# DaanVrancken/HubbardTN

Hardware: AMD Instinct MI355X
Metric: DMRG sweep time (s) + GS energy/site, 1-band Hubbard L=64 chi=1024 (lower is better)
Workload: dtype c128; 1 GPU; one-band Hubbard chain L=64 U/t=4, half filling, fZ2xSU(2)xU(1), two-site DMRG sweep (2L-3=125 bond updates) at chi=1024 (TensorKit dim units); model=one_band, L=64, chi=1024, krylovdim=30, parallelism=sector-parallel apply x1, backend=hip

## Files before the change

hubbardtn_amd/csrc/htn_svd.hip:

```cpp
#include <algorithm>
#include <utility>
#include <vector>

#include "htn_common.h"

#define JAC_THREADS 1024
#define JAC_MAXEL 8

template <int GS>
__device__ __forceinline__ double group_sum(double v) {
    v = row_sum16(v);
    if (GS == 16) return v;
    const double a = lane_bcast<0>(v) + lane_bcast<16>(v);
    const double b = lane_bcast<32>(v) + lane_bcast<48>(v);
    if (GS == 32) return (threadIdx.x & 32) ? b : a;
    return a + b;
}

template <int GS>
__device__ __forceinline__ double jacobi_pair(double2* ga, double2* gb, double2* __restrict__ va,
                                              double2* __restrict__ vb, int m, int n, int sub, double tol,
                                              bool accumulate, double zero2) {
    double2 a[JAC_MAXEL], b[JAC_MAXEL];
    double aa = 0.0, bb = 0.0, gr = 0.0, gi = 0.0;
// ... 1651 lines not shown
__device__ __forceinline__ void ring_send(const double2* __restrict__ src, double2* slot, int cnt, int tid, bool local) {
    const __amdgpu_buffer_rsrc_t rs = __builtin_amdgcn_make_buffer_rsrc((void*)slot, 0, cnt * 16, 0x00020000);
    if (local) {
        for (int idx = tid; idx < cnt; idx += RING_THREADS) {
            const double2 v = src[idx];
            ring_u4 u;
            __builtin_memcpy(&u, &v, 16);
            __builtin_amdgcn_raw_buffer_store_b128(u, rs, idx * 16, 0, 0);
        }
    } else {
        for (int idx = tid; idx < cnt; idx += RING_THREADS) {
            const double2 v = src[idx];
            ring_u4 u;
            __builtin_memcpy(&u, &v, 16);
            __builtin_amdgcn_raw_buffer_store_b128(u, rs, idx * 16, 0, 16);
        }
    }
}
__device__ __forceinline__ void ring_flag(unsigned* flag, unsigned epoch, bool local) {
    if (local) __hip_atomic_store(flag, epoch, __ATOMIC_RELAXED, __HIP_MEMORY_SCOPE_WORKGROUP);
    else __hip_atomic_store(flag, epoch, __ATOMIC_RELAXED, __HIP_MEMORY_SCOPE_AGENT);
}
__device__ __forceinline__ void ring_recv(double2* dst, const double2* slot, int cnt, int tid) {
    const __amdgpu_buffer_rsrc_t rs = __builtin_amdgcn_make_buffer_rsrc((void*)slot, 0, cnt * 16, 0x00020000);
#define RING_LD(q) const ring_u4 u##q = __builtin_amdgcn_raw_buffer_load_b128(rs, (tid + q * RING_THREADS) * 16, 0, 16)
    RING_LD(0);
    RING_LD(1);
    RING_LD(2);
    RING_LD(3);
    RING_LD(4);
    RING_LD(5);
    RING_LD(6);
    RING_LD(7);
    RING_LD(8);
#undef RING_LD
    auto put = [&](int idx, ring_u4 u) {
        if (idx < cnt) {
            double2 v;
            __builtin_memcpy(&v, &u, 16);
            dst[idx] = v;
        }
    };
    put(tid + 0 * RING_THREADS, u0);
    put(tid + 1 * RING_THREADS, u1);
    put(tid + 2 * RING_THREADS, u2);
    put(tid + 3 * RING_THREADS, u3);
    put(tid + 4 * RING_THREADS, u4);
    put(tid + 5 * RING_THREADS, u5);
    put(tid + 6 * RING_THREADS, u6);
    put(tid + 7 * RING_THREADS, u7);
    put(tid + 8 * RING_THREADS, u8);
}

template <int GS, int E, bool NORMS>
__device__ __forceinline__ double ring_rotate(double2 (&a)[E], const double2 (&b)[E], double2* b_out, double& aa, double& bb,
                                              double tol2, double zero2) {
    double gr = 0.0, gi = 0.0;
    if (NORMS) {
        double sa = 0.0, sb = 0.0;
#pragma unroll
        for (int e = 0; e < E; ++e) {
            sa = fma(a[e].x, a[e].x, fma(a[e].y, a[e].y, sa));
            sb = fma(b[e].x, b[e].x, fma(b[e].y, b[e].y, sb));
        }
        aa = group_sum<GS>(sa);
        bb = group_sum<GS>(sb);
    }
#pragma unroll
    for (int e = 0; e < E; ++e) {
        gr = fma(a[e].x, b[e].x, fma(a[e].y, b[e].y, gr));
        gi = fma(a[e].x, b[e].y, fma(-a[e].y, b[e].x, gi));
    }
    gr = group_sum<GS>(gr);
    gi = group_sum<GS>(gi);
    if (aa <= zero2 || bb <= zero2) return 0.0;
    const double g2 = fma(gr, gr, gi * gi);
    const double ab = aa * bb;
    if (g2 == 0.0) return 0.0;
    const double ratio2 = g2 * __builtin_amdgcn_rcp(ab);
    if (g2 <= tol2 * ab) return ratio2;
    const double h = bb - aa;
    const double w2 = fma(h, h, 4.0 * g2);
    const double w = w2 * __builtin_amdgcn_rsq(w2);
    double q = 2.0 * __builtin_amdgcn_rcp(fabs(h) + w);
    q = h >= 0.0 ? q : -q;
    const double c = fast_rsq(fma(q * q, g2, 1.0));
    const double cq = c * q;
    const double sr = cq * gr, si = -cq * gi;
    aa = fma(-q, g2, aa);
    bb = fma(q, g2, bb);
#pragma unroll
    for (int e = 0; e < E; ++e) {
        double2 nb;
        nb.x = fma(si, a[e].y, fma(sr, a[e].x, c * b[e].x));
        nb.y = fma(-si, a[e].x, fma(sr, a[e].y, c * b[e].y));
        b_out[GS * e] = nb;
        double x = a[e].x * c, y = a[e].y * c;
        x = fma(-sr, b[e].x, x);
        y = fma(-sr, b[e].y, y);
        a[e].x = fma(si, b[e].y, x);
        a[e].y = fma(-si, b[e].x, y);
    }
    return ratio2;
}

struct RingStamps {
    long long t[6];
};
#if defined(HTN_RING_STEP_PROF) && !defined(HTN_RING_PROF)
#error "HTN_RING_STEP_PROF needs HTN_RING_PROF (the split is stored with the phase times)"
#endif
#ifdef HTN_RING_STEP_PROF
#define RING_ST(st, i)                                                                                      \
    do {                                                                                                    \
        __builtin_amdgcn_sched_barrier(0);                                                                  \
        asm volatile("s_memtime %0\n\ts_waitcnt lgkmcnt(0)" : "=s"((st).t[i])::"memory");                  \
        __builtin_amdgcn_sched_barrier(0);                                                                  \
    } while (0)
#else
#define RING_ST(st, i) \
    do {               \
    } while (0)
#endif

template <int GS, int E>
__device__ __forceinline__ double ring_rotate_scaled(double2 (&a)[E], const double2 (&b)[E], double2* b_out, double& aa, double& bb,
                                                     double& sa, double& sb, double tol2, double zero2, RingStamps& st) {
    double gr = 0.0, gi = 0.0, gr1 = 0.0, gi1 = 0.0;
#pragma unroll
    for (int e = 0; e + 1 < E; e += 2) {
        gr = fma(a[e].x, b[e].x, fma(a[e].y, b[e].y, gr));
        gi = fma(a[e].x, b[e].y, fma(-a[e].y, b[e].x, gi));
        gr1 = fma(a[e + 1].x, b[e + 1].x, fma(a[e + 1].y, b[e + 1].y, gr1));
        gi1 = fma(a[e + 1].x, b[e + 1].y, fma(-a[e + 1].y, b[e + 1].x, gi1));
    }
    if (E & 1) {
        gr = fma(a[E - 1].x, b[E - 1].x, fma(a[E - 1].y, b[E - 1].y, gr));
        gi = fma(a[E - 1].x, b[E - 1].y, fma(-a[E - 1].y, b[E - 1].x, gi));
    }
    gr = group_sum<GS>(gr + gr1);
    gi = group_sum<GS>(gi + gi1);
    RING_ST(st, 2);
    if (aa <= zero2 || bb <= zero2) return 0.0;
    const double ss = sa * sb;
    const double g2 = ss * ss * fma(gr, gr, gi * gi);
    const double ab = aa * bb;
    if (g2 == 0.0) return 0.0;
    const double ratio2 = g2 * __builtin_amdgcn_rcp(ab);
    if (g2 <= tol2 * ab) return ratio2;
    const double h = bb - aa;
    const double w2 = fma(h, h, 4.0 * g2);
    const double w = w2 * __builtin_amdgcn_rsq(w2);
    double q = 2.0 * __builtin_amdgcn_rcp(fabs(h) + w);
    q = h >= 0.0 ? q : -q;
    const double c = fast_rsq(fma(q * q, g2, 1.0));
    aa = fma(-q, g2, aa);
    bb = fma(q, g2, bb);
    const double qb = q * sb * sb, qa = q * sa * sa;
    const double mur = qb * gr, mui = -qb * gi;
    const double nur = qa * gr, nui = qa * gi;
    sa *= c;
    sb *= c;
    RING_ST(st, 3);
#pragma unroll
    for (int e = 0; e < E; ++e) {
        double2 nb;
        nb.x = fma(-nui, a[e].y, fma(nur, a[e].x, b[e].x));
        nb.y = fma(nui, a[e].x, fma(nur, a[e].y, b[e].y));
        b_out[GS * e] = nb;
    }
#pragma unroll
    for (int e = 0; e < E; ++e) {
        double x = fma(-mur, b[e].x, a[e].x), y = fma(-mur, b[e].y, a[e].y);
        a[e].x = fma(mui, b[e].y, x);
        a[e].y = fma(-mui, b[e].x, y);
    }
    RING_ST(st, 4);
    return ratio2;
}

template <int GS, int E, bool TWO>
__device__ __forceinline__ double ring_cross(double2* T, double2* B, int nt, int nb, int tid, double tol2, double zero2, double* bnorm,
                                             double* bscale, long long* split) {
    static_assert(!TWO || GS == 16, "two partners per step need both rows of a pair in one wave");
    constexpr int mp = GS * E;
    const int grp = tid / GS, sub = tid % GS;
    const int wm = nt > nb ? nt : nb;
    double ratio = 0.0;
    if (nt == 0 || nb == 0) return ratio;
    const bool own = grp < nt;
    double2 a[E];
    double aa = 0.0, sa = 1.0;
    if (own) {
#pragma unroll
        for (int e = 0; e < E; ++e) a[e] = T[grp * mp + sub + GS * e];
        double t = 0.0;
#pragma unroll
        for (int e = 0; e < E; ++e) t = fma(a[e].x, a[e].x, fma(a[e].y, a[e].y, t));
        aa = group_sum<GS>(t);
    }
    if (grp < nb) {
        const double2* bc = B + grp * mp + sub;
        double sb = 0.0;
#pragma unroll
        for (int e = 0; e < E; ++e) {
            const double2 v = bc[GS * e];
            sb = fma(v.x, v.x, fma(v.y, v.y, sb));
        }
        sb = group_sum<GS>(sb);
        if (sub == 0) {
            bnorm[grp] = sb;
            bscale[grp] = 1.0;
        }
    }
    __syncthreads();
    constexpr int phases = TWO ? 2 : 1;
    const int hp = TWO ? (wm + 1) >> 1 : wm;
    const int row = TWO ? (grp & 1) : 0, pr = TWO ? (grp >> 1) : grp;
    (void)split;
    for (int s = 0; s < hp; ++s) {
        int jp = pr + s;
        jp = jp >= hp ? jp - hp : jp;
#ifdef HTN_RING_STEP_PROF
        long long acc[4] = {0, 0, 0, 0};
        bool all = true;
#endif
        RingStamps st;
#pragma unroll
        for (int ph = 0; ph < phases; ++ph) {
            const int j = TWO ? 2 * jp + (row ^ ph) : jp;
            st.t[4] = 0;
            RING_ST(st, 0);
            if (own && j < nb) {
                double2 b[E];
                double2* bc = B + j * mp + sub;
#pragma unroll
                for (int e = 0; e < E; ++e) b[e] = bc[GS * e];
                double bb = bnorm[j], sb = bscale[j];
                RING_ST(st, 1);
                const double rr = ring_rotate_scaled<GS, E>(a, b, bc, aa, bb, sa, sb, tol2, zero2, st);
                ratio = rr > ratio ? rr : ratio;
                if (sub == 0) {
                    bnorm[j] = bb;
                    bscale[j] = sb;
                }
            }
#ifdef HTN_RING_STEP_PROF
            if (st.t[4] == 0) all = false;
            else {
                acc[0] += st.t[1] - st.t[0];
                acc[1] += st.t[2] - st.t[1];
                acc[2] += st.t[3] - st.t[2];
                acc[3] += st.t[4] - st.t[3];
            }
#endif
            if (TWO && ph == 0) asm volatile("s_waitcnt lgkmcnt(0)" ::: "memory");
        }
#ifdef HTN_RING_STEP_PROF
        const long long tb = st.t[4];
#endif
        __syncthreads();
#ifdef HTN_RING_STEP_PROF
        RING_ST(st, 5);
        if (tid == 0 && all && tb != 0) {
            for (int q = 0; q < 4; ++q) split[q] += acc[q];
            split[4] += st.t[5] - tb;
            split[5] += 1;
            split[6] += phases;
        }
#endif
    }
    if (own) {
#pragma unroll
        for (int e = 0; e < E; ++e) T[grp * mp + sub + GS * e] = make_double2(a[e].x * sa, a[e].y * sa);
    }
    if (grp < nb) {
        const double sb = bscale[grp];
        if (sb != 1.0) {
            double2* bc = B + grp * mp + sub;
#pragma unroll
            for (int e = 0; e < E; ++e) {
                const double2 v = bc[GS * e];
                bc[GS * e] = make_double2(v.x * sb, v.y * sb);
            }
        }
    }
    __syncthreads();
    return ratio;
}

template <int GS, int E>
__device__ __forceinline__ double ring_intra(double2* T, int nt, double2* B, int nb, int tid, double tol2, double zero2) {
    constexpr int mp = GS * E;
    const int grp = tid / GS, sub = tid % GS;
    const int npT = nt + (nt & 1), npB = nb + (nb & 1), hT = npT >> 1, hB = npB >> 1;
    const int steps = (npT > npB ? npT : npB) - 1;
    double ratio = 0.0;
    for (int r = 0; r < steps; ++r) {
        double2* base = nullptr;
        int np = 0, pn = 0, p = 0;
        if (grp < hT) base = T, np = npT, pn = nt, p = grp;
        else if (grp < hT + hB) base = B, np = npB, pn = nb, p = grp - hT;
        if (base && r < np - 1) {
            const int md = np - 1;
            int i, j;
            if (p == 0) i = np - 1, j = r;
            else {
                i = r + p;
                i = i >= md ? i - md : i;
                j = r + md - p;
                j = j >= md ? j - md : j;
            }
            if (i < pn && j < pn) {
                const int lo = i < j ? i : j, hi = i < j ? j : i;
                const double rr = jacobi_pair_pad<GS, E>(base + lo * mp, base + hi * mp, sub, tol2, zero2);
                ratio = rr > ratio ? rr : ratio;
            }
        }
        __syncthreads();
    }
    return ratio;
}

#ifdef HTN_RING_PROF
__device__ long long g_ring_prof[256 * 16];
extern "C" int htn_ring_prof_dump(long long* out) {
    HIP_TRY(hipDeviceSynchronize());
    HIP_TRY(hipMemcpyFromSymbol(out, HIP_SYMBOL(g_ring_prof), sizeof(long long) * 256 * 16));
    return 0;
}
#define RING_T(var) const long long var = wall_clock64()
#define RING_ACC(slot, a, b) prof[slot] += (b) - (a)
#else
#define RING_T(var)
#define RING_ACC(slot, a, b)
#endif
struct RingArgs {
    double2* Vj;
    double2* G;
    double* S;
    const htn_svd_block* desc;
    const int* large_ids;
    const RingItem* items;
    const int* perm;
    const double* zero2;
    double2* mbox;
    unsigned* sync;
    int arrive_off, fail_off, conv_off;
    int xcc_off;
    int max_sweeps;
    int two_partner;
    double tol;
    int* info;
    int* sweeps_out;
};

template <int GS, int E>
__device__ __forceinline__ void ring_run(const RingArgs A, const RingItem it, const htn_svd_block D, double2* lds, int* s_top, int* s_bot,
                         unsigned long long* s_rbits, int* s_ok, double* s_bnorm, int* s_local) {
    constexpr int mp = GS * E;
    const int tid = threadIdx.x, lane = tid & 63, wave = tid >> 6;
    const int P = it.P, k = it.k, w = it.w, n = it.n, m = D.m;
    double2* __restrict__ X = A.Vj + D.v_off;
    const int slot_elems = w * mp;
    double2* bufT = lds;
    double2* bufB = lds + slot_elems;
    unsigned* flags = A.sync;
    unsigned* fail = A.sync + A.fail_off;
    const double zero2 = A.zero2[it.li];
    const double tol2 = A.tol * A.tol, thr = fmax(tol2, 0.1 * A.tol);
    auto ncols = [&](int q) {
        const int c = n - q * w;
        return c < 0 ? 0 : (c > w ? w : c);
    };
    if (tid < P) {
        s_top[tid] = 2 * tid;
        s_bot[tid] = 2 * tid + 1;
    }
    if (tid == 0) {
        *s_ok = 1;
        int local = 0;
        if (P > 1 && A.xcc_off >= 0) {
            unsigned xcc;
            asm volatile("s_getreg_b32 %0, hwreg(HW_REG_XCC_ID)" : "=s"(xcc));
            xcc = (xcc & 0xfu) + 1u;
            unsigned* xw = A.sync + A.xcc_off + it.g0;
            __hip_atomic_store(xw + k, xcc, __ATOMIC_RELAXED, __HIP_MEMORY_SCOPE_AGENT);
            local = 1;
            for (int q = 0; q < P && local >= 0; ++q) {
                if (!ring_wait_ge(xw + q, 1u, fail)) local = -1;
                else if (__hip_atomic_load(xw + q, __ATOMIC_RELAXED, __HIP_MEMORY_SCOPE_AGENT) != xcc) local = local > 0 ? 0 : local;
            }
            if (local < 0) *s_ok = 0;
        }
        *s_local = local > 0 ? 1 : 0;
    }
    __syncthreads();
    const bool local = *s_local != 0;
    {
        const int gsx = m <= 16 * JAC_MAXEL ? 16 : (m <= 32 * JAC_MAXEL ? 32 : 64);
        const int ldx = gsx * ((m + gsx - 1) / gsx);
        for (int side = 0; side < 2; ++side) {
            const int q = side ? s_bot[k] : s_top[k];
            double2* buf = side ? bufB : bufT;
            const int cnt = ncols(q) * mp;
            for (int idx = tid; idx < cnt; idx += RING_THREADS) {
                const int c = idx / mp, i = idx - c * mp;
                buf[idx] = i < m ? X[(int64_t)(q * w + c) * ldx + i] : make_double2(0.0, 0.0);
            }
        }
    }
    __syncthreads();
#ifdef HTN_RING_PROF
    long long prof[16] = {0, 0, 0, 0, 0, 0, 0, 0, 0, 0, 0, 0, 0, 0, 0, 0};
    const long long prof_t0 = wall_clock64();
    long long prof_c0;
    asm volatile("s_memtime %0\n\ts_waitcnt lgkmcnt(0)" : "=s"(prof_c0)::"memory");
#endif
    long long* split = nullptr;
#ifdef HTN_RING_STEP_PROF
    split = prof + 8;
#endif
    int sweeps = 0;
    bool done = n < 2, ok = *s_ok != 0;
    const int rounds = 2 * P - 1;
    while (!done && ok && sweeps < A.max_sweeps) {
        double ratio = 0.0;
        for (int r = 0; r < rounds && ok; ++r) {
            const unsigned epoch = (unsigned)(sweeps * rounds + r + 1);
            const int par = (int)(epoch & 1u);
            const int nt = ncols(s_top[k]), nb = ncols(s_bot[k]);
            RING_T(p0);
            double rr;
            if constexpr (GS == 16) {
                if (A.two_partner) rr = ring_cross<GS, E, true>(bufT, bufB, nt, nb, tid, tol2, zero2, s_bnorm, s_bnorm + RING_THREADS / 16, split);
                else rr = ring_cross<GS, E, false>(bufT, bufB, nt, nb, tid, tol2, zero2, s_bnorm, s_bnorm + RING_THREADS / 16, split);
            } else {
                rr = ring_cross<GS, E, false>(bufT, bufB, nt, nb, tid, tol2, zero2, s_bnorm, s_bnorm + RING_THREADS / 16, split);
            }
            ratio = rr > ratio ? rr : ratio;
            RING_T(p1);
            RING_ACC(0, p0, p1);
            if (P < 2) continue;
            double2* box = A.mbox + it.mbox;
            if (k == 0) ring_send(bufB, box + (int64_t)((1 * 2 + 0) * 2 + par) * slot_elems, nb * mp, tid, local);
            else {
                if (k < P - 1) ring_send(bufT, box + (int64_t)(((k + 1) * 2 + 0) * 2 + par) * slot_elems, nt * mp, tid, local);
                ring_send(bufB, box + (int64_t)(((k - 1) * 2 + 1) * 2 + par) * slot_elems, nb * mp, tid, local);
            }
            asm volatile("s_waitcnt vmcnt(0)" ::: "memory");
            __syncthreads();
            RING_T(p2);
            RING_ACC(1, p1, p2);
            if (tid == 0) {
                if (k == 0) ring_flag(flags + (it.g0 + 1) * 2 + 0, epoch, local);
                else {
                    if (k < P - 1) ring_flag(flags + (it.g0 + k + 1) * 2 + 0, epoch, local);
                    ring_flag(flags + (it.g0 + k - 1) * 2 + 1, epoch, local);
                }
                const int t_last = s_top[P - 1], b0 = s_bot[0];
                for (int q = P - 1; q >= 2; --q) s_top[q] = s_top[q - 1];
                s_top[1] = b0;
                for (int q = 0; q + 1 < P; ++q) s_bot[q] = s_bot[q + 1];
                s_bot[P - 1] = t_last;
                bool good = true;
                if (k > 0) good = ring_wait_ge(flags + (it.g0 + k) * 2 + 0, epoch, fail);
                if (good && k < P - 1) good = ring_wait_ge(flags + (it.g0 + k) * 2 + 1, epoch, fail);
                if (!good) *s_ok = 0;
            }
            if (k == P - 1) {
                double2* t = bufT;
                bufT = bufB;
                bufB = t;
            }
            __syncthreads();
            RING_T(p3);
            RING_ACC(2, p2, p3);
            ok = *s_ok != 0;
            if (ok) {
                const double2* mine = box + (int64_t)(k * 4) * slot_elems;
                if (k > 0) ring_recv(bufT, mine + (int64_t)(0 * 2 + par) * slot_elems, ncols(s_top[k]) * mp, tid);
                if (k < P - 1) ring_recv(bufB, mine + (int64_t)(1 * 2 + par) * slot_elems, ncols(s_bot[k]) * mp, tid);
            }
            __syncthreads();
            RING_T(p4);
            RING_ACC(3, p3, p4);
        }
        if (!ok) break;
        RING_T(p5);
        {
            const double rr = ring_intra<GS, E>(bufT, ncols(s_top[k]), bufB, ncols(s_bot[k]), tid, tol2, zero2);
            ratio = rr > ratio ? rr : ratio;
        }
        RING_T(p6);
        RING_ACC(4, p5, p6);
        if (tid == 0) *s_rbits = 0ull;
        __syncthreads();
        {
            const unsigned long long key = wave_max_u64((unsigned long long)__double_as_longlong(ratio));
            if (lane == 0 && key) atomicMax(s_rbits, key);
        }
        __syncthreads();
        if (tid == 0) {
            unsigned long long* conv = (unsigned long long*)(A.sync + A.conv_off) + (int64_t)it.li * A.max_sweeps + sweeps;
            unsigned* arrive = A.sync + A.arrive_off + it.li * A.max_sweeps + sweeps;
            unsigned long long mx = *s_rbits;
            if (P > 1) {
                const unsigned long long old = __hip_atomic_fetch_max(conv, mx, __ATOMIC_RELAXED, __HIP_MEMORY_SCOPE_AGENT);
                asm volatile("s_waitcnt vmcnt(0)" ::: "memory");
                (void)old;
                __hip_atomic_fetch_add(arrive, 1u, __ATOMIC_RELAXED, __HIP_MEMORY_SCOPE_AGENT);
                if (ring_wait_ge(arrive, (unsigned)P, fail)) mx = __hip_atomic_load(conv, __ATOMIC_RELAXED, __HIP_MEMORY_SCOPE_AGENT);
                else *s_ok = 0;
            }
            *s_rbits = mx;
        }
        __syncthreads();
        ok = *s_ok != 0;
        ++sweeps;
        done = __longlong_as_double((long long)*s_rbits) <= thr;
        __syncthreads();
        RING_T(p7);
        RING_ACC(5, p6, p7);
    }
#ifdef HTN_RING_PROF
    if (tid == 0 && blockIdx.x < 256) {
        prof[6] = wall_clock64() - prof_t0;
        prof[7] = (local ? 1000000 : 0) + sweeps * 1000 + P;
        long long prof_c1;
        asm volatile("s_memtime %0\n\ts_waitcnt lgkmcnt(0)" : "=s"(prof_c1)::"memory");
        prof[15] = prof_c1 - prof_c0;
        for (int q = 0; q < 16; ++q) g_ring_prof[blockIdx.x * 16 + q] = prof[q];
    }
#endif
    double2* __restrict__ g = A.G + D.g_off;
    const int* __restrict__ pc = A.perm + it.li * 64 * JAC_MAXEL;
    for (int side = 0; side < 2; ++side) {
        const double2* buf = side ? bufB : bufT;
        const int q = side ? s_bot[k] : s_top[k];
        const int nc = ncols(q);
        for (int c = wave; c < nc; c += RING_THREADS / 64) {
            const int col = q * w + c;
            double sn = 0.0;
            for (int i = lane; i < m; i += 64) {
                const double2 x = buf[c * mp + i];
                sn += x.x * x.x + x.y * x.y;
                g[(int64_t)col * m + pc[i]] = x;
            }
            sn = wave_sum(sn);
            if (lane == 0) A.S[D.s_off + col] = sqrt(sn);
        }
    }
    for (int col = n + k * (RING_THREADS / 64) + wave; col < D.n; col += P * (RING_THREADS / 64)) {
        for (int i = lane; i < m; i += 64) g[(int64_t)col * m + i] = make_double2(0.0, 0.0);
        if (lane == 0) A.S[D.s_off + col] = 0.0;
    }
    if (k == 0 && tid == 0) {
        A.info[A.large_ids[it.li]] = (done && ok) ? sweeps : -(sweeps > 0 ? sweeps : 1);
        A.sweeps_out[it.li] = ok ? sweeps + ((local || P == 1) ? 1000 : 0) : 0;
        __threadfence_system();
    }
}

__global__ __launch_bounds__(RING_THREADS) void k_jacobi_ring(RingArgs A) {
    extern __shared__ double2 g_lds[];
    __shared__ int s_top[RING_MAX_P], s_bot[RING_MAX_P];
    __shared__ unsigned long long s_rbits;
    __shared__ int s_ok, s_local;
    __shared__ double s_bnorm[2 * (RING_THREADS / 16)];
    const RingItem it = A.items[blockIdx.x];
    if (it.P <= 0) return;
    const htn_svd_block D = A.desc[A.large_ids[it.li]];
    const int m = D.m;
    const int gs = ring_gs(m), E = ring_e(m);
#define RING_CASE(GSV, EV) \
    case EV: ring_run<GSV, EV>(A, it, D, g_lds, s_top, s_bot, &s_rbits, &s_ok, s_bnorm, &s_local); break;
    if (gs == 16) {
        switch (E) {
            RING_CASE(16, 1) RING_CASE(16, 2) RING_CASE(16, 3) RING_CASE(16, 4) RING_CASE(16, 5) RING_CASE(16, 6) RING_CASE(16, 7)
            RING_CASE(16, 8) RING_CASE(16, 9) RING_CASE(16, 10) RING_CASE(16, 11) RING_CASE(16, 12) RING_CASE(16, 13)
            RING_CASE(16, 14) RING_CASE(16, 15)
            default: ring_run<16, 16>(A, it, D, g_lds, s_top, s_bot, &s_rbits, &s_ok, s_bnorm, &s_local);
        }
    } else {
        switch (E) {
            RING_CASE(64, 5) RING_CASE(64, 6) RING_CASE(64, 7)
            default: ring_run<64, 8>(A, it, D, g_lds, s_top, s_bot, &s_rbits, &s_ok, s_bnorm, &s_local);
        }
    }
#undef RING_CASE
}

struct JacScratch {
    int device = -1;
    int cu_count = 0;
    int xcd_local = 0;
    HtnBuf dev{HTN_BUF_DEVICE};
    HtnBuf pinned{HTN_BUF_PINNED};
    HtnBuf flags{HTN_BUF_MAPPED};
    HtnBuf ring_sync{HTN_BUF_DEVICE, false};
    HtnBuf ring_items{HTN_BUF_DEVICE, false};
    HtnBuf ring_items_h{HTN_BUF_PINNED};
    HtnBuf ring_mbox{HTN_BUF_DEVICE};
    HtnBuf qr_box{HTN_BUF_DEVICE};
    HtnBuf tall_dev{HTN_BUF_DEVICE};
    HtnBuf tall_pin{HTN_BUF_PINNED};
    HtnBuf tall_flags{HTN_BUF_MAPPED};
    hipStream_t aux = nullptr;
    hipEvent_t ev_fork = nullptr, ev_join = nullptr, ev_sweep[2] = {nullptr, nullptr};
    ~JacScratch() {
        if (device >= 0) (void)hipSetDevice(device);
        if (aux) {
            (void)hipStreamSynchronize(aux);
            (void)hipStreamDestroy(aux);
        }
        for (hipEvent_t ev : {ev_fork, ev_join, ev_sweep[0], ev_sweep[1]})
            if (ev) (void)hipEventDestroy(ev);
    }
};
static HtnStreamRegistry<JacScratch> g_js_res;

void htn_svd_release_stream(hipStream_t st) { g_js_res.release(st); }

static int js_get(hipStream_t st, JacScratch** out) {
    return g_js_res.get(st, out, [](JacScratch& js) -> int {
        HIP_TRY(hipDeviceGetAttribute(&js.cu_count, hipDeviceAttributeMultiprocessorCount, js.device));
        HIP_TRY(hipStreamCreateWithFlags(&js.aux, hipStreamNonBlocking));
        HIP_TRY(hipEventCreateWithFlags(&js.ev_fork, hipEventDisableTiming));
        HIP_TRY(hipEventCreateWithFlags(&js.ev_join, hipEventDisableTiming));
        HIP_TRY(hipEventCreateWithFlags(&js.ev_sweep[0], hipEventDisableTiming));
        HIP_TRY(hipEventCreateWithFlags(&js.ev_sweep[1], hipEventDisableTiming));
        return 0;
    });
}

struct JacTournament {
    std::vector<JacPairItem> items;
    std::vector<size_t> off;
    int n_rounds() const { return (int)off.size() - 1; }
    unsigned round_size(int r) const { return (unsigned)(off[r + 1] - off[r]); }
// ... 202 lines not shown
            for (int y = 1; y < nx; ++y)
                if (lane_used[y] < lane_used[x]) x = y;
            if (lane_used[x] + blks[q].P > lane_cap) continue;
            puts.push_back({(int)q, x, lane_used[x]});
            lane_used[x] += blks[q].P;
            placed[q] = 1;
            --left;
        }
        int depth = 0;
        for (int y = 0; y < nx; ++y) depth = std::max(depth, lane_used[y]);
        const int grid = depth * nx;
        plan->items.resize((size_t)first + grid, RingItem{0, 0, 0, 0, 0, 0, 0});
        for (const Put& pt : puts) {
            const Blk& B = blks[pt.q];
            for (int k = 0; k < B.P; ++k)
                plan->items[(size_t)first + (size_t)(pt.s0 + k) * nx + pt.x] = {B.li, k, B.P, B.w, c.n_eff[B.li], plan->wgs,
                                                                                 plan->mbox_elems};
            plan->mbox_elems += (int64_t)B.P * 4 * B.w * B.mp;
            plan->wgs += B.P;
        }
        plan->batches.push_back({first, grid});
    }
    return true;
}

static int launch_qr_large(const JacCall& c, JacScratch& js, const JacCoreBufs& B, int n_xcd) {
    const int nl = c.nl();
    int max_m0 = 0, min_m0 = 1 << 30, max_n0 = 0;
    for (int b : c.large) {
        max_m0 = std::max(max_m0, (int)c.desc_host[b].pad);
        min_m0 = std::min(min_m0, (int)c.desc_host[b].pad);
        max_n0 = std::max(max_n0, (int)c.desc_host[b].m);
    }
    const size_t qr_panel_elems = (size_t)16 * (((max_m0 + 15) & ~15) + 1);
    const bool coop = ((min_m0 + 15) & ~15) <= 256 && qr_panel_elems * sizeof(double2) + 65536 + 30720 <= 163840;
    const size_t qr_lds = qr_panel_elems * sizeof(double2) + (coop ? 65536 : 0);
    static const bool qr_single = htn_env_flag("HTN_QR_SINGLE");
    static const int env_nw = getenv("HTN_QR_NW") ? atoi(getenv("HTN_QR_NW")) : 0;
    int NW = qr_single ? 1 : ((max_n0 >= 160 || js.xcd_local) ? 4 : 1);
    if (env_nw > 0 && !qr_single) NW = std::min(env_nw, 4);
    const int cus = std::max(1, std::min(js.cu_count > 0 ? js.cu_count : 256, 256));
    const int qnx = (NW > 1 && n_xcd > 1) ? n_xcd : 1;
    const int nl_pad = (nl + qnx - 1) / qnx * qnx;
    NW = std::max(1, std::min(NW, cus / std::max(nl_pad, 1)));
    if (NW > 1 && js.qr_box.reserve((size_t)nl * QR_BOX_BYTES)) return 1;
    const int qgrid_nx = NW > 1 ? qnx : 1;
    hipLaunchKernelGGL(k_qr_large, dim3((NW > 1 ? nl_pad : nl) * NW), dim3(JAC_THREADS), qr_lds, c.st, c.G, c.Vj, c.desc, B.d_ids,
                       B.d_perm, B.d_zero, c.cut2, B.d_rank, NW, (char*)js.qr_box.p, B.d_qsync, nl, qgrid_nx,
                       coop ? (int)qr_panel_elems : 0);
    return 0;
}

static int run_ring(const JacCall& c, JacScratch& js, const JacCoreBufs& B, const RingPlan& plan, int n_xcd, bool two_partner,
                    int32_t* sweeps_used) {
    const int nl = c.nl(), n_wg = plan.wgs, n_items = (int)plan.items.size();
    const int arrive_off = 2 * n_wg, fail_off = arrive_off + nl * c.max_sweeps, xcc_off = fail_off + 1;
    const int conv_off = (xcc_off + n_wg + 3) & ~3;
    const size_t sync_bytes = ((size_t)conv_off * 4 + (size_t)nl * c.max_sweeps * 8 + 15) & ~(size_t)15;
    if (js.ring_sync.reserve(sync_bytes)) return 1;
    if (js.ring_mbox.reserve(sizeof(double2) * (size_t)std::max<int64_t>(plan.mbox_elems, 1))) return 1;
    if (js.ring_items.reserve(sizeof(RingItem) * n_items) || js.ring_items_h.reserve(sizeof(RingItem) * n_items)) return 1;
    memcpy(js.ring_items_h.p, plan.items.data(), sizeof(RingItem) * n_items);
    for (int li = 0; li < nl; ++li) B.h_ring_sw[li] = 0;
    HIP_TRY(hipMemcpyAsync(js.ring_items.p, js.ring_items_h.p, sizeof(RingItem) * n_items, hipMemcpyHostToDevice, c.st));
    HIP_TRY(hipMemsetAsync(js.ring_sync.p, 0, sync_bytes, c.st));
    RingArgs ra;
    ra.Vj = c.Vj, ra.G = c.G, ra.S = c.S, ra.desc = c.desc, ra.large_ids = B.d_ids;
    ra.perm = B.d_perm, ra.zero2 = B.d_zero, ra.mbox = (double2*)js.ring_mbox.p, ra.sync = (unsigned*)js.ring_sync.p;
    ra.arrive_off = arrive_off, ra.fail_off = fail_off, ra.conv_off = conv_off, ra.max_sweeps = c.max_sweeps, ra.tol = c.tol;
    ra.xcc_off = xcc_off;
    ra.two_partner = two_partner ? 1 : 0;
    ra.info = c.info_dev, ra.sweeps_out = B.d_ring_sw;
    for (auto& bt : plan.batches) {
        ra.items = (const RingItem*)js.ring_items.p + bt.first;
        hipLaunchKernelGGL(k_jacobi_ring, dim3((unsigned)bt.second), dim3(RING_THREADS), 2 * RING_PANEL_ELEMS * sizeof(double2),
                           c.st, ra);
    }
    HIP_TRY(hipGetLastError());
    HIP_TRY(hipStreamWaitEvent(c.st, js.ev_join, 0));
    HIP_TRY(htn_stream_spin(c.st));
    int used = 0;
    for (int li = 0; li < nl; ++li) {
        if (B.h_rank[li] < 0) return fail_msg("htn_jacobi_svd_z: a hand-off of the multi-workgroup QR timed out");
        if (B.h_ring_sw[li] <= 0 && c.n_eff[li] >= 2)
            return fail_msg("htn_jacobi_svd_z: a hand-off of the ring Jacobi kernel timed out");
        used = std::max(used, (int)B.h_ring_sw[li] % 1000);
    }
    int all_local = n_xcd > 1 ? 1 : 0;
    for (int li = 0; li < nl; ++li)
        if (c.n_eff[li] >= 2 && B.h_ring_sw[li] < 1000) all_local = 0;
    js.xcd_local = all_local;
    if (sweeps_used) *sweeps_used = used;
    return 0;
}

static int run_pair_visits(const JacCall& c, JacScratch& js, const JacCoreBufs& B, const JacTournament& T, int hint,
                           int32_t* sweeps_used) {
    const int nl = c.nl();
    int max_mp = 0;
    for (int b : c.large) max_mp = std::max(max_mp, jac_padded_rows(c.desc_host[b].m));
    const size_t gram_lds_bytes = (size_t)(16 * (max_mp + 1) + JG_GU_ELEMS) * sizeof(double2);
    const double thr = std::max(c.tol * c.tol, 0.1 * c.tol);
    const int used = jacobi_sweep_pipeline(c.max_sweeps, hint, js.ev_sweep, B.h_active, c.st, [&](int sweep) {
        for (int r = 0; r < T.n_rounds(); ++r)
            if (T.round_size(r))
                hipLaunchKernelGGL(k_jacobi_pairs_gram, dim3(T.round_size(r)), dim3(256), gram_lds_bytes, c.st, c.Vj, c.desc,
                                   B.d_ids, B.d_items + T.off[r], B.d_zero, B.d_ratio, B.d_done, c.tol, 1);
        hipLaunchKernelGGL(k_jacobi_check, dim3(1), dim3(64), 0, c.st, B.d_ratio, B.d_done, B.d_sw, nl, thr, B.d_active + sweep);
    });
    if (used < 0) return 1;
    if (sweeps_used) *sweeps_used = used;
    HIP_TRY(hipStreamWaitEvent(c.st, js.ev_join, 0));
    hipLaunchKernelGGL(k_jacobi_finish, dim3(nl), dim3(JAC_THREADS), 0, c.st, c.G, (const double2*)c.Vj, c.S, c.desc, B.d_ids,
                       B.d_perm, B.d_sw, B.d_done, c.info_dev);
    HIP_TRY(hipGetLastError());
    HIP_TRY(htn_stream_spin(c.st));
    return 0;
}

static int jacobi_svd_core(void* G, void* Vj, double* S, const htn_svd_block* desc, const htn_svd_block* desc_host,
                           int32_t n_blocks, int32_t max_m_host, int32_t max_sweeps, double tol, int32_t* info_dev,
                           const htn_svd_opts* opts, void* stream, const int* skip_dev, const unsigned char* skip_host) {
    if (n_blocks <= 0) return 0;
    if (max_m_host > 64 * JAC_MAXEL) return fail_msg("htn_jacobi_svd_z: block taller than 512 rows");
    const double rank_cut = opts && opts->rank_cut > 0.0 ? opts->rank_cut : 0.0;
    JacCall c = {(double2*)G, (double2*)Vj, S, desc, desc_host, n_blocks, max_sweeps, tol, rank_cut * rank_cut,
                 opts && opts->split_elems > 0 ? opts->split_elems : 0, info_dev, (hipStream_t)stream, {}, {}};
    int32_t* sweeps_used = opts ? opts->sweeps_used : nullptr;
    if (jac_set_kernel_attributes()) return 1;
    c.large = classify_large(desc_host, n_blocks, c.split);
    if (sweeps_used) *sweeps_used = 0;
    if (c.large.empty()) {
        hipLaunchKernelGGL(k_jacobi_svd, dim3(n_blocks), dim3(JAC_THREADS), JAC_LDS_ELEMS * sizeof(double2), c.st, c.G, c.Vj, S,
                           desc, max_sweeps, tol, info_dev, JAC_LDS_ELEMS, skip_dev, c.cut2);
        HIP_TRY(hipGetLastError());
        return 0;
    }
    const int nl = c.nl();
    size_t n_items_max = 0;
    for (int b : c.large) {
        const int nb = (desc_host[b].n + JAC_PANEL - 1) / JAC_PANEL, nbp = nb + (nb & 1);
        n_items_max += (size_t)(nbp - 1) * (nbp / 2) + (nb + 1) / 2;
        c.n_eff.push_back(desc_host[b].n);
    }
    JacScratch* jsp = nullptr;
    JacCoreBufs B;
    if (js_get(c.st, &jsp) || carve_core_scratch(*jsp, nl, n_blocks, max_sweeps, n_items_max, &B)) return 1;
    JacScratch& js = *jsp;
    for (int b = 0; b < n_blocks; ++b) B.h_slot[b] = skip_host && skip_host[b] ? nl : -1;
    for (int li = 0; li < nl; ++li) B.h_slot[c.large[li]] = li;
    for (int li = 0; li < nl; ++li) B.h_ids[li] = c.large[li];
    for (int k = 0; k <= max_sweeps; ++k) B.h_active[k] = 1;
    HIP_TRY(hipMemcpyAsync(B.d_ids, B.h_ids, sizeof(int) * (nl + n_blocks), hipMemcpyHostToDevice, c.st));
    HIP_TRY(hipMemsetAsync(B.d_ratio, 0, 16 * (size_t)nl + sizeof(unsigned) * (QR_SYNC_WORDS * (size_t)nl + 8), c.st));
    static const bool force_pairs = htn_env_flag("HTN_SVD_PAIRS");
    static const bool no_xcd = htn_env_flag("HTN_RING_NO_XCD");
    const bool ring_two_partner = htn_env_flag("HTN_RING_TWO_PARTNER");
    const int n_xcd = (!no_xcd && js.cu_count > 0 && js.cu_count % 8 == 0) ? 8 : 1;
    const int ring_cap = std::max(1, std::min(js.cu_count > 0 ? js.cu_count : 256, 256));
    RingPlan plan;
    JacTournament T;
    bool use_ring = !force_pairs && plan_ring(c, n_xcd, ring_cap, &plan);
    if (c.cut2 <= 0.0 && !use_ring) {
        T = jacobi_tournament(c.n_eff.data(), nl);
        if (upload_tournament(T, B.h_items, B.d_items, c.st)) return 1;
    }
    HIP_TRY(hipEventRecord(js.ev_fork, c.st));
    HIP_TRY(hipStreamWaitEvent(js.aux, js.ev_fork, 0));
    hipLaunchKernelGGL(k_jacobi_svd, dim3(n_blocks), dim3(JAC_THREADS), JAC_LDS_ELEMS * sizeof(double2), js.aux, c.G, c.Vj, S,
                       desc, max_sweeps, tol, info_dev, JAC_LDS_ELEMS, (const int*)B.d_slot, c.cut2);
    HIP_TRY(hipEventRecord(js.ev_join, js.aux));
    if (launch_qr_large(c, js, B, n_xcd)) return 1;
    if (c.cut2 > 0.0) {
        HIP_TRY(hipEventRecord(js.ev_sweep[0], c.st));
        HIP_TRY(htn_event_spin(js.ev_sweep[0]));
        for (int li = 0; li < nl; ++li) c.n_eff[li] = std::min(c.n_eff[li], (int)B.h_rank[li]);
        if (use_ring) use_ring = plan_ring(c, n_xcd, ring_cap, &plan);
        if (!use_ring) {
            T = jacobi_tournament(c.n_eff.data(), nl);
            if (upload_tournament(T, B.h_items, B.d_items, c.st)) return 1;
        }
    }
    if (use_ring) return run_ring(c, js, B, plan, n_xcd, ring_two_partner, sweeps_used);
    return run_pair_visits(c, js, B, T, opts && opts->sweeps_hint > 0 ? opts->sweeps_hint : 0, sweeps_used);
}

static int jacobi_svd_tall(void* G, void* Vj, double* S, const htn_svd_block* desc, const htn_svd_block* desc_host,
                           int32_t n_blocks, int32_t max_m_rest, int32_t max_sweeps, double tol, int32_t* info_dev,
                           const htn_svd_opts* opts, void* stream, const std::vector<int>& tall) {
    const int nt = (int)tall.size();
    hipStream_t st = (hipStream_t)stream;
    JacScratch* jsp = nullptr;
    if (js_get(st, &jsp)) return 1;
    JacScratch& js = *jsp;
    std::vector<int> n_cols(nt);
    for (int li = 0; li < nt; ++li) n_cols[li] = desc_host[tall[li]].n;
    const JacTournament T = jacobi_tournament(n_cols.data(), nt);
    const size_t n_items = T.items.size();
    const size_t off_skip = 0, off_ids = off_skip + sizeof(int) * n_blocks;
    const size_t off_zero = (off_ids + sizeof(int) * nt + 7) / 8 * 8, off_part = off_zero + sizeof(double) * nt;
    const size_t off_ratio = off_part + sizeof(double) * nt * TALL_PARTS, off_done = off_ratio + 8 * (size_t)nt;
    const size_t off_sw = off_done + sizeof(int) * nt, off_items = (off_sw + sizeof(int) * nt + 31) / 32 * 32;
    const size_t flag_elems = (size_t)std::max(max_sweeps, 0) + 1;
    if (js.tall_dev.reserve(off_items + sizeof(JacPairItem) * std::max<size_t>(n_items, 1))) return 1;
    if (js.tall_pin.reserve(sizeof(JacPairItem) * std::max<size_t>(n_items, 1) + sizeof(int) * (n_blocks + nt))) return 1;
    if (js.tall_flags.reserve(sizeof(int) * flag_elems)) return 1;
    char* d = (char*)js.tall_dev.p;
    int* d_skip = (int*)(d + off_skip);
    int* d_ids = (int*)(d + off_ids);
    double* d_zero = (double*)(d + off_zero);
    double* d_part = (double*)(d + off_part);
    unsigned long long* d_ratio = (unsigned long long*)(d + off_ratio);
    int* d_done = (int*)(d + off_done);
    int* d_sw = (int*)(d + off_sw);
    JacPairItem* d_items = (JacPairItem*)(d + off_items);
    JacPairItem* h_items = (JacPairItem*)js.tall_pin.p;
    int* h_skip = (int*)((char*)js.tall_pin.p + sizeof(JacPairItem) * std::max<size_t>(n_items, 1));
    int* h_ids = h_skip + n_blocks;
    volatile int* h_active = (volatile int*)js.tall_flags.p;
    int* d_active = (int*)js.tall_flags.dev;
    std::vector<unsigned char> skip(n_blocks, 0);
    for (int li = 0; li < nt; ++li) skip[tall[li]] = 1;
    for (int b = 0; b < n_blocks; ++b) h_skip[b] = skip[b] ? 0 : -1;
    for (int li = 0; li < nt; ++li) h_ids[li] = tall[li];
    for (size_t k = 0; k < flag_elems; ++k) h_active[k] = 1;
    HIP_TRY(hipMemcpyAsync(d_skip, h_skip, sizeof(int) * (n_blocks + nt), hipMemcpyHostToDevice, st));
    if (upload_tournament(T, h_items, d_items, st)) return 1;
    HIP_TRY(hipMemsetAsync(d_ratio, 0, 16 * (size_t)nt, st));
    int core_used = 0;
    if (nt < n_blocks) {
        if (jacobi_svd_core(G, Vj, S, desc, desc_host, n_blocks, max_m_rest, max_sweeps, tol, info_dev, opts, stream, d_skip,
                            skip.data()))
            return 1;
        if (opts && opts->sweeps_used) core_used = *opts->sweeps_used;
    }
    int max_n = 1;
// ... 83 lines not shown
```

Before: 422.0 ms.

## Send rotated ring columns straight from registers and split arrival waits per half

```diff
diff --git a/hubbardtn_amd/csrc/htn_svd.hip b/hubbardtn_amd/csrc/htn_svd.hip
--- a/hubbardtn_amd/csrc/htn_svd.hip
+++ b/hubbardtn_amd/csrc/htn_svd.hip
@@ -1727,6 +1727,62 @@
     put(tid + 8 * RING_THREADS, u8);
 }
 
+__device__ __forceinline__ void ring_store16(double2 x, __amdgpu_buffer_rsrc_t rs, int elem, bool local) {
+    ring_u4 u;
+    __builtin_memcpy(&u, &x, 16);
+    if (local) __builtin_amdgcn_raw_buffer_store_b128(u, rs, elem * 16, 0, 0);
+    else __builtin_amdgcn_raw_buffer_store_b128(u, rs, elem * 16, 0, 16);
+}
+template <int GS, int E>
+__device__ __forceinline__ void ring_send_col(const double2 (&v)[E], double s, __amdgpu_buffer_rsrc_t rs, int off, bool local) {
+#pragma unroll
+    for (int e = 0; e < E; ++e) ring_store16(make_double2(v[e].x * s, v[e].y * s), rs, off + GS * e, local);
+}
+template <int GS, int E>
+__device__ __forceinline__ void ring_recv_cols(double2* dst, const double2* slot, int nc, int g, int ng, int sub, double* norm,
+                                               double* scale) {
+    constexpr int mp = GS * E;
+    constexpr bool PAIRS = GS == 64 || E <= 9;
+    const __amdgpu_buffer_rsrc_t rs = __builtin_amdgcn_make_buffer_rsrc((void*)slot, 0, nc * mp * 16, 0x00020000);
+    auto put = [&](int c, const ring_u4 (&u)[E]) {
+        if (c < nc) {
+            double2* col = dst + c * mp + sub;
+            double t = 0.0;
+#pragma unroll
+            for (int e = 0; e < E; ++e) {
+                double2 v;
+                __builtin_memcpy(&v, &u[e], 16);
+                t = fma(v.x, v.x, fma(v.y, v.y, t));
+                col[GS * e] = v;
+            }
+            t = group_sum<GS>(t);
+            if (sub == 0) {
+                norm[c] = t;
+                if (scale) scale[c] = 1.0;
+            }
+        }
+    };
+    for (int c0 = g; c0 < nc; c0 += (PAIRS ? 2 : 1) * ng) {
+        ring_u4 u0[E];
+#pragma unroll
+        for (int e = 0; e < E; ++e) u0[e] = __builtin_amdgcn_raw_buffer_load_b128(rs, (c0 * mp + sub + GS * e) * 16, 0, 16);
+        if constexpr (PAIRS) {
+            const int c1 = c0 + ng;
+            ring_u4 u1[E];
+#pragma unroll
+            for (int e = 0; e < E; ++e) u1[e] = __builtin_amdgcn_raw_buffer_load_b128(rs, (c1 * mp + sub + GS * e) * 16, 0, 16);
+            put(c0, u0);
+            put(c1, u1);
+        } else put(c0, u0);
+    }
+}
+struct RingOut {
+    __amdgpu_buffer_rsrc_t slot_t, slot_b;
+    bool send_t;
+    bool keep_t;
+    bool local;
+};
+
 template <int GS, int E, bool NORMS>
 __device__ __forceinline__ double ring_rotate(double2 (&a)[E], const double2 (&b)[E], double2* b_out, double& aa, double& bb,
                                               double tol2, double zero2) {
@@ -1798,9 +1854,11 @@
     } while (0)
 #endif
 
-template <int GS, int E>
+template <int GS, int E, bool OUT = false>
 __device__ __forceinline__ double ring_rotate_scaled(double2 (&a)[E], const double2 (&b)[E], double2* b_out, double& aa, double& bb,
-                                                     double& sa, double& sb, double tol2, double zero2, RingStamps& st) {
+                                                     double& sa, double& sb, double tol2, double zero2, RingStamps& st,
+                                                     __amdgpu_buffer_rsrc_t out_rs = __amdgpu_buffer_rsrc_t(), int out_off = 0,
+                                                     bool out_local = false, bool* sent = nullptr) {
     double gr = 0.0, gi = 0.0, gr1 = 0.0, gi1 = 0.0;
 #pragma unroll
     for (int e = 0; e + 1 < E; e += 2) {
@@ -1837,27 +1895,46 @@
     sa *= c;
     sb *= c;
     RING_ST(st, 3);
-#pragma unroll
-    for (int e = 0; e < E; ++e) {
-        double2 nb;
-        nb.x = fma(-nui, a[e].y, fma(nur, a[e].x, b[e].x));
-        nb.y = fma(nui, a[e].x, fma(nur, a[e].y, b[e].y));
-        b_out[GS * e] = nb;
-    }
-#pragma unroll
-    for (int e = 0; e < E; ++e) {
-        double x = fma(-mur, b[e].x, a[e].x), y = fma(-mur, b[e].y, a[e].y);
-        a[e].x = fma(mui, b[e].y, x);
-        a[e].y = fma(-mui, b[e].x, y);
+    if constexpr (OUT) {
+        *sent = true;
+#pragma unroll
+        for (int e = 0; e < E; ++e) {
+            double2 nb;
+            nb.x = fma(-nui, a[e].y, fma(nur, a[e].x, b[e].x));
+            nb.y = fma(nui, a[e].x, fma(nur, a[e].y, b[e].y));
+            ring_store16(make_double2(nb.x * sb, nb.y * sb), out_rs, out_off + GS * e, out_local);
+        }
+#pragma unroll
+        for (int e = 0; e < E; ++e) {
+            double x = fma(-mur, b[e].x, a[e].x), y = fma(-mur, b[e].y, a[e].y);
+            a[e].x = fma(mui, b[e].y, x);
+            a[e].y = fma(-mui, b[e].x, y);
+        }
+    } else {
+#pragma unroll
+        for (int e = 0; e < E; ++e) {
+            double2 nb;
+            nb.x = fma(-nui, a[e].y, fma(nur, a[e].x, b[e].x));
+            nb.y = fma(nui, a[e].x, fma(nur, a[e].y, b[e].y));
+            b_out[GS * e] = nb;
+        }
+#pragma unroll
+        for (int e = 0; e < E; ++e) {
+            double x = fma(-mur, b[e].x, a[e].x), y = fma(-mur, b[e].y, a[e].y);
+            a[e].x = fma(mui, b[e].y, x);
+            a[e].y = fma(-mui, b[e].x, y);
+        }
     }
     RING_ST(st, 4);
     return ratio2;
 }
 
-template <int GS, int E, bool TWO>
+template <int GS, int E, bool TWO, bool SEND>
 __device__ __forceinline__ double ring_cross(double2* T, double2* B, int nt, int nb, int tid, double tol2, double zero2, double* bnorm,
-                                             double* bscale, long long* split) {
+                                             double* bscale, const double* tnorm, bool have_t, bool have_b, const RingOut& out,
+                                             long long* split) {
     static_assert(!TWO || GS == 16, "two partners per step need both rows of a pair in one wave");
+    static_assert(!(TWO && SEND), "the two-partner step keeps the staged send");
     constexpr int mp = GS * E;
     const int grp = tid / GS, sub = tid % GS;
     const int wm = nt > nb ? nt : nb;
@@ -1869,12 +1946,15 @@
     if (own) {
 #pragma unroll
         for (int e = 0; e < E; ++e) a[e] = T[grp * mp + sub + GS * e];
-        double t = 0.0;
-#pragma unroll
-        for (int e = 0; e < E; ++e) t = fma(a[e].x, a[e].x, fma(a[e].y, a[e].y, t));
-        aa = group_sum<GS>(t);
-    }
-    if (grp < nb) {
+        if (have_t) aa = tnorm[grp];
+        else {
+            double t = 0.0;
+#pragma unroll
+            for (int e = 0; e < E; ++e) t = fma(a[e].x, a[e].x, fma(a[e].y, a[e].y, t));
+            aa = group_sum<GS>(t);
+        }
+    }
+    if (!have_b && grp < nb) {
         const double2* bc = B + grp * mp + sub;
         double sb = 0.0;
 #pragma unroll
@@ -1888,12 +1968,12 @@
             bscale[grp] = 1.0;
         }
     }
-    __syncthreads();
+    if (!have_b) __syncthreads();
     constexpr int phases = TWO ? 2 : 1;
     const int hp = TWO ? (wm + 1) >> 1 : wm;
     const int row = TWO ? (grp & 1) : 0, pr = TWO ? (grp >> 1) : grp;
     (void)split;
-    for (int s = 0; s < hp; ++s) {
+    for (int s = 0; s < (SEND ? hp - 1 : hp); ++s) {
         int jp = pr + s;
         jp = jp >= hp ? jp - hp : jp;
 #ifdef HTN_RING_STEP_PROF
@@ -1944,6 +2024,33 @@
             split[6] += phases;
         }
 #endif
+    }
+    if constexpr (SEND) {
+        int jp = pr + hp - 1;
+        jp = jp >= hp ? jp - hp : jp;
+        RingStamps st;
+        if (grp < hp && jp < nb) {
+            double2 b[E];
+            const double2* bc = B + jp * mp + sub;
+#pragma unroll
+            for (int e = 0; e < E; ++e) b[e] = bc[GS * e];
+            double bb = bnorm[jp], sb = bscale[jp];
+            bool sent = false;
+            if (own) {
+                const double rr = ring_rotate_scaled<GS, E, true>(a, b, nullptr, aa, bb, sa, sb, tol2, zero2, st, out.slot_b,
+                                                                  jp * mp + sub, out.local, &sent);
+                ratio = rr > ratio ? rr : ratio;
+            }
+            if (!sent) ring_send_col<GS, E>(b, sb, out.slot_b, jp * mp + sub, out.local);
+        }
+        if (own) {
+            if (out.send_t) ring_send_col<GS, E>(a, sa, out.slot_t, grp * mp + sub, out.local);
+            if (out.keep_t) {
+#pragma unroll
+                for (int e = 0; e < E; ++e) T[grp * mp + sub + GS * e] = make_double2(a[e].x * sa, a[e].y * sa);
+            }
+        }
+        return ratio;
     }
     if (own) {
 #pragma unroll
@@ -2025,6 +2132,7 @@
     int xcc_off;
     int max_sweeps;
     int two_partner;
+    int staged_send;
     double tol;
     int* info;
     int* sweeps_out;
@@ -2032,7 +2140,7 @@
 
 template <int GS, int E>
 __device__ __forceinline__ void ring_run(const RingArgs A, const RingItem it, const htn_svd_block D, double2* lds, int* s_top, int* s_bot,
-                         unsigned long long* s_rbits, int* s_ok, double* s_bnorm, int* s_local) {
+                         unsigned long long* s_rbits, int* s_ok, double* s_bnorm, int* s_local, unsigned* s_arr) {
     constexpr int mp = GS * E;
     const int tid = threadIdx.x, lane = tid & 63, wave = tid >> 6;
     const int P = it.P, k = it.k, w = it.w, n = it.n, m = D.m;
@@ -2054,6 +2162,7 @@
     }
     if (tid == 0) {
         *s_ok = 1;
+        s_arr[0] = s_arr[1] = 0u;
         int local = 0;
         if (P > 1 && A.xcc_off >= 0) {
             unsigned xcc;
@@ -2099,6 +2208,9 @@
     int sweeps = 0;
     bool done = n < 2, ok = *s_ok != 0;
     const int rounds = 2 * P - 1;
+    const bool direct = A.staged_send == 0;
+    double* const s_bscale = s_bnorm + RING_THREADS / 16;
+    double* const s_tnorm = s_bnorm + 2 * (RING_THREADS / 16);
     while (!done && ok && sweeps < A.max_sweeps) {
         double ratio = 0.0;
         for (int r = 0; r < rounds && ok; ++r) {
@@ -2106,27 +2218,39 @@
             const int par = (int)(epoch & 1u);
             const int nt = ncols(s_top[k]), nb = ncols(s_bot[k]);
             RING_T(p0);
-            double rr;
-            if constexpr (GS == 16) {
-                if (A.two_partner) rr = ring_cross<GS, E, true>(bufT, bufB, nt, nb, tid, tol2, zero2, s_bnorm, s_bnorm + RING_THREADS / 16, split);
-                else rr = ring_cross<GS, E, false>(bufT, bufB, nt, nb, tid, tol2, zero2, s_bnorm, s_bnorm + RING_THREADS / 16, split);
-            } else {
-                rr = ring_cross<GS, E, false>(bufT, bufB, nt, nb, tid, tol2, zero2, s_bnorm, s_bnorm + RING_THREADS / 16, split);
-            }
+            double2* box = A.mbox + it.mbox;
+            double2* const to_t = box + (int64_t)(((k + 1) * 2 + 0) * 2 + par) * slot_elems;
+            double2* const to_b = k == 0 ? box + (int64_t)((1 * 2 + 0) * 2 + par) * slot_elems
+                                         : box + (int64_t)(((k - 1) * 2 + 1) * 2 + par) * slot_elems;
+            const bool send_t = k > 0 && k < P - 1;
+            const bool have_t = direct && r > 0 && k > 0, have_b = direct && r > 0 && k < P - 1;
+            const bool reg_send = direct && !(GS == 16 && A.two_partner) && P > 1 && nt > 0 && nb > 0;
+            RingOut out;
+            out.slot_t = __builtin_amdgcn_make_buffer_rsrc((void*)to_t, 0, (reg_send && send_t) ? nt * mp * 16 : 0, 0x00020000);
+            out.slot_b = __builtin_amdgcn_make_buffer_rsrc((void*)to_b, 0, reg_send ? nb * mp * 16 : 0, 0x00020000);
+            out.send_t = send_t, out.keep_t = !send_t, out.local = local;
+            double rr = 0.0;
+            if (reg_send) rr = ring_cross<GS, E, false, true>(bufT, bufB, nt, nb, tid, tol2, zero2, s_bnorm, s_bscale, s_tnorm, have_t, have_b, out, split);
+            else if (GS == 16 && A.two_partner) {
+                if constexpr (GS == 16)
+                    rr = ring_cross<GS, E, true, false>(bufT, bufB, nt, nb, tid, tol2, zero2, s_bnorm, s_bscale, s_tnorm, have_t, have_b, out, split);
+            } else rr = ring_cross<GS, E, false, false>(bufT, bufB, nt, nb, tid, tol2, zero2, s_bnorm, s_bscale, s_tnorm, have_t, have_b, out, split);
             ratio = rr > ratio ? rr : ratio;
             RING_T(p1);
             RING_ACC(0, p0, p1);
             if (P < 2) continue;
-            double2* box = A.mbox + it.mbox;
-            if (k == 0) ring_send(bufB, box + (int64_t)((1 * 2 + 0) * 2 + par) * slot_elems, nb * mp, tid, local);
-            else {
-                if (k < P - 1) ring_send(bufT, box + (int64_t)(((k + 1) * 2 + 0) * 2 + par) * slot_elems, nt * mp, tid, local);
-                ring_send(bufB, box + (int64_t)(((k - 1) * 2 + 1) * 2 + par) * slot_elems, nb * mp, tid, local);
-            }
+            if (!reg_send) {
+                if (send_t) ring_send(bufT, to_t, nt * mp, tid, local);
+                ring_send(bufB, to_b, nb * mp, tid, local);
+            }
+            const int in_top = k == 0 ? s_top[0] : (k == 1 ? s_bot[0] : s_top[k - 1]);
+            const int in_bot = k < P - 1 ? s_bot[k + 1] : s_top[P - 1];
             asm volatile("s_waitcnt vmcnt(0)" ::: "memory");
             __syncthreads();
             RING_T(p2);
             RING_ACC(1, p1, p2);
+            const int half = k == 0 ? 1 : (k == P - 1 ? 0 : wave >> 2);
+            const bool both = k > 0 && k < P - 1;
             if (tid == 0) {
                 if (k == 0) ring_flag(flags + (it.g0 + 1) * 2 + 0, epoch, local);
                 else {
@@ -2138,28 +2262,53 @@
                 s_top[1] = b0;
                 for (int q = 0; q + 1 < P; ++q) s_bot[q] = s_bot[q + 1];
                 s_bot[P - 1] = t_last;
-                bool good = true;
-                if (k > 0) good = ring_wait_ge(flags + (it.g0 + k) * 2 + 0, epoch, fail);
-                if (good && k < P - 1) good = ring_wait_ge(flags + (it.g0 + k) * 2 + 1, epoch, fail);
-                if (!good) *s_ok = 0;
+                if (!direct) {
+                    bool good = true;
+                    if (k > 0) good = ring_wait_ge(flags + (it.g0 + k) * 2 + 0, epoch, fail);
+                    if (good && k < P - 1) good = ring_wait_ge(flags + (it.g0 + k) * 2 + 1, epoch, fail);
+                    if (!good) *s_ok = 0;
+                }
             }
             if (k == P - 1) {
                 double2* t = bufT;
                 bufT = bufB;
                 bufB = t;
             }
-            __syncthreads();
-            RING_T(p3);
-            RING_ACC(2, p2, p3);
-            ok = *s_ok != 0;
-            if (ok) {
-                const double2* mine = box + (int64_t)(k * 4) * slot_elems;
-                if (k > 0) ring_recv(bufT, mine + (int64_t)(0 * 2 + par) * slot_elems, ncols(s_top[k]) * mp, tid);
-                if (k < P - 1) ring_recv(bufB, mine + (int64_t)(1 * 2 + par) * slot_elems, ncols(s_bot[k]) * mp, tid);
-            }
-            __syncthreads();
-            RING_T(p4);
-            RING_ACC(3, p3, p4);
+            if (!direct) {
+                __syncthreads();
+                RING_T(p3);
+                RING_ACC(2, p2, p3);
+                ok = *s_ok != 0;
+                if (ok) {
+                    const double2* mine = box + (int64_t)(k * 4) * slot_elems;
+                    if (k > 0) ring_recv(bufT, mine + (int64_t)(0 * 2 + par) * slot_elems, ncols(s_top[k]) * mp, tid);
+                    if (k < P - 1) ring_recv(bufB, mine + (int64_t)(1 * 2 + par) * slot_elems, ncols(s_bot[k]) * mp, tid);
+                }
+                __syncthreads();
+                RING_T(p4);
+                RING_ACC(3, p3, p4);
+            } else {
+                if (tid == (both ? half * (RING_THREADS / 2) : 0)) {
+                    const bool good = ring_wait_ge(flags + (it.g0 + k) * 2 + half, epoch, fail);
+                    if (!good) *s_ok = 0;
+                    __hip_atomic_store(s_arr + half, good ? epoch : ~0u, __ATOMIC_RELEASE, __HIP_MEMORY_SCOPE_WORKGROUP);
+                }
+                unsigned seen;
+                while ((seen = __hip_atomic_load(s_arr + half, __ATOMIC_ACQUIRE, __HIP_MEMORY_SCOPE_WORKGROUP)) < epoch)
+                    __builtin_amdgcn_s_sleep(1);
+                RING_T(p3);
+                RING_ACC(2, p2, p3);
+                if (seen != ~0u) {
+                    const double2* mine = box + (int64_t)(k * 4 + half * 2 + par) * slot_elems;
+                    const int ngt = RING_THREADS / GS, ng = both ? ngt / 2 : ngt, grp = tid / GS;
+                    ring_recv_cols<GS, E>(half ? bufB : bufT, mine, ncols(half ? in_bot : in_top), both ? grp % ng : grp, ng, tid % GS,
+                                          half ? s_bnorm : s_tnorm, half ? s_bscale : nullptr);
+                }
+                __syncthreads();
+                RING_T(p4);
+                RING_ACC(3, p3, p4);
+                ok = *s_ok != 0;
+            }
         }
         if (!ok) break;
         RING_T(p5);
@@ -2242,25 +2391,26 @@
     __shared__ int s_top[RING_MAX_P], s_bot[RING_MAX_P];
     __shared__ unsigned long long s_rbits;
     __shared__ int s_ok, s_local;
-    __shared__ double s_bnorm[2 * (RING_THREADS / 16)];
+    __shared__ double s_bnorm[3 * (RING_THREADS / 16)];
+    __shared__ unsigned s_arr[2];
     const RingItem it = A.items[blockIdx.x];
     if (it.P <= 0) return;
     const htn_svd_block D = A.desc[A.large_ids[it.li]];
     const int m = D.m;
     const int gs = ring_gs(m), E = ring_e(m);
 #define RING_CASE(GSV, EV) \
-    case EV: ring_run<GSV, EV>(A, it, D, g_lds, s_top, s_bot, &s_rbits, &s_ok, s_bnorm, &s_local); break;
+    case EV: ring_run<GSV, EV>(A, it, D, g_lds, s_top, s_bot, &s_rbits, &s_ok, s_bnorm, &s_local, s_arr); break;
     if (gs == 16) {
         switch (E) {
             RING_CASE(16, 1) RING_CASE(16, 2) RING_CASE(16, 3) RING_CASE(16, 4) RING_CASE(16, 5) RING_CASE(16, 6) RING_CASE(16, 7)
             RING_CASE(16, 8) RING_CASE(16, 9) RING_CASE(16, 10) RING_CASE(16, 11) RING_CASE(16, 12) RING_CASE(16, 13)
             RING_CASE(16, 14) RING_CASE(16, 15)
-            default: ring_run<16, 16>(A, it, D, g_lds, s_top, s_bot, &s_rbits, &s_ok, s_bnorm, &s_local);
+            default: ring_run<16, 16>(A, it, D, g_lds, s_top, s_bot, &s_rbits, &s_ok, s_bnorm, &s_local, s_arr);
         }
     } else {
         switch (E) {
             RING_CASE(64, 5) RING_CASE(64, 6) RING_CASE(64, 7)
-            default: ring_run<64, 8>(A, it, D, g_lds, s_top, s_bot, &s_rbits, &s_ok, s_bnorm, &s_local);
+            default: ring_run<64, 8>(A, it, D, g_lds, s_top, s_bot, &s_rbits, &s_ok, s_bnorm, &s_local, s_arr);
         }
     }
 #undef RING_CASE
@@ -2569,7 +2719,7 @@
 }
 
 static int run_ring(const JacCall& c, JacScratch& js, const JacCoreBufs& B, const RingPlan& plan, int n_xcd, bool two_partner,
-                    int32_t* sweeps_used) {
+                    bool staged_send, int32_t* sweeps_used) {
     const int nl = c.nl(), n_wg = plan.wgs, n_items = (int)plan.items.size();
     const int arrive_off = 2 * n_wg, fail_off = arrive_off + nl * c.max_sweeps, xcc_off = fail_off + 1;
     const int conv_off = (xcc_off + n_wg + 3) & ~3;
@@ -2587,6 +2737,7 @@
     ra.arrive_off = arrive_off, ra.fail_off = fail_off, ra.conv_off = conv_off, ra.max_sweeps = c.max_sweeps, ra.tol = c.tol;
     ra.xcc_off = xcc_off;
     ra.two_partner = two_partner ? 1 : 0;
+    ra.staged_send = staged_send ? 1 : 0;
     ra.info = c.info_dev, ra.sweeps_out = B.d_ring_sw;
     for (auto& bt : plan.batches) {
         ra.items = (const RingItem*)js.ring_items.p + bt.first;
@@ -2672,6 +2823,7 @@
     HIP_TRY(hipMemsetAsync(B.d_ratio, 0, 16 * (size_t)nl + sizeof(unsigned) * (QR_SYNC_WORDS * (size_t)nl + 8), c.st));
     static const bool force_pairs = htn_env_flag("HTN_SVD_PAIRS");
     static const bool no_xcd = htn_env_flag("HTN_RING_NO_XCD");
+    static const bool ring_staged = htn_env_flag("HTN_RING_STAGED_SEND");
     const bool ring_two_partner = htn_env_flag("HTN_RING_TWO_PARTNER");
     const int n_xcd = (!no_xcd && js.cu_count > 0 && js.cu_count % 8 == 0) ? 8 : 1;
     const int ring_cap = std::max(1, std::min(js.cu_count > 0 ? js.cu_count : 256, 256));
@@ -2698,7 +2850,7 @@
             if (upload_tournament(T, B.h_items, B.d_items, c.st)) return 1;
         }
     }
-    if (use_ring) return run_ring(c, js, B, plan, n_xcd, ring_two_partner, sweeps_used);
+    if (use_ring) return run_ring(c, js, B, plan, n_xcd, ring_two_partner, ring_staged, sweeps_used);
     return run_pair_visits(c, js, B, T, opts && opts->sweeps_hint > 0 ? opts->sweeps_hint : 0, sweeps_used);
 }
 
```

Result: faster. 407.7 ms, median of 6 (-3.4%).
